# crlotwhite/pytorch_hmm

Hardware: AMD Instinct MI355X
Metric: frames/sec forward-backward+Viterbi, B=32 T=2000 N=128, 1/2/4/8 GPU (higher is better)
Workload: dtype f32; 1 GPU; HMMPyTorch forward_backward + viterbi_decode; batch_per_gpu=32, global_batch=32, seq_len=2000, num_states=128, transition=left_to_right(0.7), world_size_seen=1, parallelism=batch-sharded x1, streams=2, gather=False, hip_graph=False, step_pipelining=per-op streams, no per-step join, transition_plan=True, fb_kernel=chains + posterior followers in one launch, viterbi_kernel=chains + log leaders + decode followers in one launch

## Files before the change

include/hmm355.h:

```cpp
#ifndef HMM355_H
#define HMM355_H

#include <stddef.h>
#include <stdint.h>

#ifdef __cplusplus
extern "C" {
#endif

#define HMM355_OK 0
#define HMM355_E_ARG (-1)
#define HMM355_E_STATES (-2)
#define HMM355_E_SHAPE (-3)
#define HMM355_E_WORKSPACE (-4)
#define HMM355_E_DURATION (-5)

#define HMM355_OBS_PROB 0
#define HMM355_OBS_LOG 1

#define HMM355_FB_POSTERIOR 1u
#define HMM355_FB_FORWARD 2u
#define HMM355_FB_BACKWARD 4u
#define HMM355_FB_PAIR 0x100u
#define HMM355_FB_PLAN_BANDED 0x200u

const char* hmm355_strerror(int code);
int hmm355_version(void);

size_t hmm355_fb_workspace_bytes(int B, int T, int N);
int hmm355_fb_workspace_layout(int B, int T, int N, size_t* offsets);
int hmm355_forward_backward_ex_f32(const float* obs, int obs_mode, const float* log_P,
                                   const float* log_p0, const float* log_beta_T, int B, int T, int N,
                                   unsigned out_mask, float* posterior, float* forward,
                                   float* backward, float* loglik, float* lik_ref, void* workspace,
                                   size_t workspace_bytes, void* stream);
int hmm355_forward_backward_f32(const float* obs, int obs_mode, const float* log_P,
                                const float* log_p0, int B, int T, int N, unsigned out_mask,
                                float* posterior, float* forward, float* backward,
                                float* loglik, float* lik_ref, void* workspace,
                                size_t workspace_bytes, void* stream);

int hmm355_fb_adjoint_f32(const float* E, const float* log_P, const float* src_w,
                          const float* scale_w, const float* src_z, const float* scale_z,
                          int B, int T, int N, float* W, float* P, void* stream);

size_t hmm355_plan_bytes(int N);
int hmm355_plan_f32(const float* log_P, int N, void* plan, void* stream);
// ... 143 lines not shown
```

pytorch_hmm_amd/_native.py:

```python
import ctypes
import os

import torch

_HERE = os.path.dirname(os.path.abspath(__file__))
LIB_PATH = os.environ.get("HMM355_LIB", os.path.join(_HERE, "lib", "libhmm355.so"))

OBS_PROB = 0
OBS_LOG = 1
FB_POSTERIOR = 1
FB_PAIR = 0x100
FB_PLAN_BANDED = 0x200
VIT_PLAN_BANDED = 0x1
VIT_PLAN_DENSE = 0x2
PLAN_DENSE = 0x1
FORM_GENERAL = 0x1
FORM_SERIAL_WALK = 0x2
FB_FORWARD = 2
FB_BACKWARD = 4
NARROW_MAX_STATES = 256
WIDE_MAX_STATES = 4096
DTW_SYMMETRIC, DTW_ASYMMETRIC, DTW_RABINER_JUANG = 0, 1, 2
DTW_PATH = 0x1
CTC_ALPHA, CTC_BETA, CTC_VITERBI = 0x1, 0x2, 0x4
CTC_MAX_TARGET = 2048

EXPORTS = (
    "hmm355_strerror", "hmm355_version",
    "hmm355_fb_workspace_bytes", "hmm355_fb_workspace_layout", "hmm355_forward_backward_f32",
    "hmm355_forward_backward_ex_f32",
    "hmm355_viterbi_workspace_bytes", "hmm355_viterbi_workspace_bytes_ex", "hmm355_viterbi_f32",
    "hmm355_gmm_workspace_bytes", "hmm355_gmm_diag_logprob_f32",
    "hmm355_hsmm_workspace_bytes", "hmm355_hsmm_viterbi_f32", "hmm355_hsmm_workspace_bytes_ex",
    "hmm355_hsmm_viterbi_ex_f32",
    "hmm355_tv_fb_workspace_bytes", "hmm355_tv_forward_backward_f32", "hmm355_tv_forward_backward_ex_f32",
# ... 130 lines not shown
```

pytorch_hmm_amd/csrc/capi.hip:

```cpp
#include "common.h"

HMM355_API int hmm355_version(void) { return 4; }

HMM355_API const char* hmm355_strerror(int code) {
  switch (code) {
    case HMM355_OK: return "ok";
    case HMM355_E_ARG: return "invalid argument (null pointer, negative size or unknown mode)";
    case HMM355_E_STATES: return "number of states outside the op's range (HMM recursions [1, 256], their *_wide forms [1, 4096], HSMM [1, 1024], CTC target length [1, 2048])";
    case HMM355_E_SHAPE: return "invalid shape (T < 1, a DTW matrix without rows or columns, or size overflow)";
    case HMM355_E_WORKSPACE: return "workspace too small";
    case HMM355_E_DURATION: return "HSMM max_duration outside [1, 1024]";
    default: break;
  }
  if (code > 0) return hipGetErrorString(static_cast<hipError_t>(code));
  return "unknown hmm355 error";
}
```

pytorch_hmm_amd/csrc/fb.hip:

```cpp
#include <atomic>

#include "recur.h"
#include "post.h"
#include "fbpair.h"

namespace hmm355 {

template <int NP>
hipError_t launch_fb(const RecArgs& fa, const RecArgs& fb, const PostArgs& pa, bool prep, hipStream_t st, int nfollow);
template <int NP>
hipError_t launch_fb_pair(const PairArgs& pa, int B, hipStream_t st);
__global__ void __launch_bounds__(256) row_max_kernel(const float* __restrict__ lo, int N, size_t rows,
                                                      float* __restrict__ m) {
  const int l = threadIdx.x & 63;
  const size_t nw = ((size_t)gridDim.x * blockDim.x) >> 6;
  for (size_t row = ((size_t)blockIdx.x * blockDim.x + threadIdx.x) >> 6; row < rows; row += nw) {
    const float* src = lo + row * N;
    float v = -INFINITY;
    for (int j = l; j < N; j += 64) v = fmaxf(v, src[j]);
    v = wave_max_dpp2(v);
    if (l == 0) m[row] = (v > -INFINITY && v < INFINITY) ? v : 0.f;
  }
}

// ... 129 lines not shown
    const hipError_t e1 = hipGetLastError();
    if (e1 != hipSuccess) return (int)e1;
    rmax = w.rmax;
  }
  RecArgs fa{obs, log_P, log_p0, w.U, w.LA, loglik, B, T, N, obs_mode, NP, band, nullptr, nullptr, nullptr, rmax, nullptr};
  RecArgs fb{obs, log_P, log_p0, w.V, w.LB, nullptr, B, T, N, obs_mode, NP, band, binit, bscale, nullptr, rmax, nullptr};
  fa.cs = w.CA;
  fb.cs = w.CB;
  hipStream_t st0 = static_cast<hipStream_t>(stream);
  if ((out_mask & HMM355_FB_PAIR) && plan && band && NP <= 128 && !log_beta_T &&
      (size_t)T * NP * sizeof(float) < ((size_t)1 << 31)) {
    PairArgs pa{fa, fb, posterior, forward, backward, lik_ref, out_mask};
    const hipError_t e = NP == 64 ? launch_fb_pair<64>(pa, B, st0) : launch_fb_pair<128>(pa, B, st0);
    return e == hipSuccess ? HMM355_OK : (int)e;
  }
  fa.out_exp = (out_mask & HMM355_FB_FORWARD) ? forward : nullptr;
  fb.out_exp = (out_mask & HMM355_FB_BACKWARD) ? backward : nullptr;
  int nfollow = 0;
  if ((out_mask & HMM355_FB_PLAN_BANDED) && plan && (out_mask & HMM355_FB_POSTERIOR) && 3 * B <= fb_device_cus() &&
      (size_t)T * NP * 4 < ((size_t)1 << 31)) {
    fa.pub = fb.pub = w.pub;
    fa.lik_ref = lik_ref;
    nfollow = HMM355_FBF > 0 ? HMM355_FBF : (4 * B <= fb_device_cus() ? 2 : 1);
  }
  PostArgs pa{w.U, w.V, w.LA, w.LB, posterior, forward, backward, lik_ref, B, T, N,
              out_mask & (HMM355_FB_POSTERIOR)};
  hipError_t e;
  switch (NP) {
    case 64: e = launch_fb<64>(fa, fb, pa, plan == nullptr, st, nfollow); break;
    case 128: e = launch_fb<128>(fa, fb, pa, plan == nullptr, st, nfollow); break;
    default: e = launch_fb<256>(fa, fb, pa, plan == nullptr, st, nfollow); break;
  }
  return e == hipSuccess ? HMM355_OK : (int)e;
}

HMM355_API int hmm355_forward_backward_ex_f32(const float* obs, int obs_mode, const float* log_P,
                                              const float* log_p0, const float* log_beta_T, int B, int T, int N,
                                              unsigned out_mask, float* posterior, float* forward, float* backward,
                                              float* loglik, float* lik_ref, void* workspace,
                                              size_t workspace_bytes, void* stream) {
  return hmm355_forward_backward_plan_f32(obs, obs_mode, log_P, log_p0, nullptr, log_beta_T, B, T, N, out_mask,
                                          posterior, forward, backward, loglik, lik_ref, workspace,
                                          workspace_bytes, stream);
}

HMM355_API int hmm355_forward_backward_f32(const float* obs, int obs_mode, const float* log_P,
// ... 9 lines not shown
```

pytorch_hmm_amd/csrc/follow.h:

```cpp
#pragma once
#include "recur.h"
#include "post.h"

namespace hmm355 {

constexpr long long kFollowGiveUp = 20000000;

__device__ __forceinline__ void fstamp(int k) {
  if (kStamp && threadIdx.x == 0)
    g_rec_stamps[((size_t)blockIdx.x * 16 % kStampWaves) * 8 + k] = __builtin_amdgcn_s_memrealtime();
}

__device__ __forceinline__ void follow_poll(const int* p, int need, int* slot, unsigned token, int cap) {
  int have = poll_count(p, token, cap), last = have;
  long long t0 = __builtin_amdgcn_s_memrealtime();
  while (have < need) {
    __builtin_amdgcn_s_sleep(20);
    have = poll_count(p, token, cap);
    const long long now = __builtin_amdgcn_s_memrealtime();
    if (have != last) {
      last = have;
      t0 = now;
    } else if (now - t0 > kFollowGiveUp) {
      have = -1;
      break;
    }
  }
  *slot = have;
}

template <int NP>
__device__ __forceinline__ void vit_lead(const RecArgs& a, int b) {
  const int T = a.T, N = a.N, nblocks = (T + 15) / 16;
  if (!a.lobuf || nblocks <= 4 || (kFAbl & (fabl::kNoFollowers | fabl::kNoLogLeaders))) return;
  const int tid = threadIdx.x, nt = blockDim.x;
  const size_t off = (size_t)b * T * N;
  const float* src = a.obs + off;
  float* dst = const_cast<float*>(a.lobuf) + off;
  int* cnt = const_cast<int*>(a.lready) + b * kPubStride;
  const __amdgpu_buffer_rsrc_t rs = make_rsrc(dst, (size_t)T * N * 4);
  const bool vec = (N & 3) == 0 && ((reinterpret_cast<uintptr_t>(src) | reinterpret_cast<uintptr_t>(dst)) & 15) == 0;
  constexpr int kRound = 8;
  for (int k0 = 4; k0 < nblocks; k0 += kRound) {
    const int k1 = k0 + kRound < nblocks ? k0 + kRound : nblocks;
    const int e0 = 16 * k0 * N, e1 = (16 * k1 < T ? 16 * k1 : T) * N;
    if (vec) {
      for (int i0 = e0 / 4 + tid; i0 < e1 / 4; i0 += 4 * nt) {
        float4 v[4];
#pragma unroll
        for (int k = 0; k < 4; ++k) {
          const int i = i0 + k * nt;
          v[k] = reinterpret_cast<const float4*>(src)[i < e1 / 4 ? i : i0];
        }
#pragma unroll
        for (int k = 0; k < 4; ++k) {
          const int i = i0 + k * nt;
          const float4 o = make_float4(logcr_fast(v[k].x + 1e-8f, g_logcr_tab), logcr_fast(v[k].y + 1e-8f, g_logcr_tab),
                                       logcr_fast(v[k].z + 1e-8f, g_logcr_tab), logcr_fast(v[k].w + 1e-8f, g_logcr_tab));
          if (i < e1 / 4) __builtin_amdgcn_raw_buffer_store_b128(__builtin_bit_cast(u32x4_t, o), rs, i * 16, 0, kAuxSc1);
        }
      }
    } else {
      for (int i = e0 + tid; i < e1; i += nt)
        __builtin_amdgcn_raw_buffer_store_b32(__builtin_bit_cast(unsigned, logcr_fast(src[i] + 1e-8f, g_logcr_tab)), rs,
                                              i * 4, 0, kAuxSc1);
    }
    asm volatile("s_waitcnt vmcnt(0)" ::: "memory");
    __syncthreads();
    if (tid == 0) publish_count(cnt, k1, a.token);
  }
}

__host__ __device__ constexpr int follow_g(int NP) { return 1024 / NP < 8 ? 1024 / NP : 8; }
inline size_t vit_follow_lds_bytes(int T, int NP) {
  const size_t nc = (T + kChunk - 1) / kChunk;
  return align_up(nc * NP, 16) + (size_t)follow_g(NP) * kChunk * NP + align_up(nc, 4) * 4 + 64;
}

template <int NP>
__device__ __forceinline__ void vit_decode_follow(const RecArgs& a, int b, float* ldsf) {
  const int T = a.T, N = a.N, nblocks = (T + 15) / 16, nc = (T + kChunk - 1) / kChunk;
  const int tid = threadIdx.x, w = __builtin_amdgcn_readfirstlane(tid >> 6), l = tid & 63, nw = blockDim.x >> 6;
  uint8_t* lds = reinterpret_cast<uint8_t*>(ldsf);
  uint8_t* gm = lds;
  uint8_t* stg = gm + align_up((size_t)nc * NP, 16);
  int* send = reinterpret_cast<int*>(stg + (size_t)follow_g(NP) * kChunk * NP);
  int* ctl = send + align_up((size_t)nc, 4);
  int64_t* sb = a.states + (size_t)b * T;
  auto invalid = [&]() {
    for (int t = tid; t < T; t += blockDim.x) sb[t] = -1;
    if (tid == 0 && a.final_score) a.final_score[b] = __builtin_bit_cast(float, 0x7fc00000u);
  };
  fstamp(0);
  if (kFAbl & fabl::kNoFollowers) return;
  if (rec_band_code<kVit, NP>(a) == 0) {
    invalid();
    return;
  }
  const int* pubp = a.pub + b * kPubStride;
  const __amdgpu_buffer_rsrc_t psi_rs = make_rsrc(a.psi + (size_t)b * T * NP, (size_t)T * NP);
  constexpr int G = follow_g(NP);
  int have = 0;
  int next = 0;
  auto wait_for = [&](int need) -> bool {
    if (tid == 0) follow_poll(pubp, need, ctl, a.token, nblocks + 1);
    __syncthreads();
    const int v = ctl[0];
    __syncthreads();
    if (v < 0) return false;
    have = v;
    return true;
  };
  uint8_t* const pbase = a.path + (size_t)b * nc * NP * kChunk;
  auto compose = [&](int c_end) {
    while (next < c_end) {
      const int cnt = c_end - next < G ? c_end - next : G;
      const int per = kChunk * NP / 16;
      for (int idx = tid; idx < cnt * per; idx += blockDim.x) {
        const int g = idx / per, pc = idx - g * per;
        const int t = (next + g) * kChunk + pc / (NP / 16);
        const u32x4_t v = t < T ? __builtin_amdgcn_raw_buffer_load_b128(psi_rs, (t * NP) + 16 * (pc % (NP / 16)), 0, kAuxSc1)
                                : u32x4_t{0u, 0u, 0u, 0u};
        *reinterpret_cast<u32x4_t*>(stg + (size_t)g * kChunk * NP + 16 * pc) = v;
      }
      __syncthreads();
      const int g = tid / NP, j = tid % NP;
      if (g < cnt) {
        const int c = next + g;
        const int t_lo = c * kChunk, t_hi = (t_lo + kChunk < T ? t_lo + kChunk : T) - 1;
        const int len = t_hi - t_lo;
        const uint8_t* pr = stg + (size_t)g * kChunk * NP;
        int st = j < N ? j : 0;
        unsigned acc[kChunk / 4];
        static_for<0, kChunk>([&](auto KK) {
          constexpr int k = kChunk - 1 - decltype(KK)::value;
          if constexpr ((k & 3) == 3) acc[k >> 2] = (unsigned)st << 24;
          else acc[k >> 2] |= (unsigned)st << (8 * (k & 3));
          if constexpr (k >= 1) {
            const int nx = pr[k * NP + st];
            st = k <= len ? nx : st;
          }
        });
        gm[(size_t)c * NP + j] = pr[st];
        uint8_t* dst = pbase + ((size_t)c * NP + j) * kChunk;
#pragma unroll
        for (int q = 0; q < kChunk / 16; ++q)
          *reinterpret_cast<u32x4_t*>(dst + 16 * q) = u32x4_t{acc[4 * q], acc[4 * q + 1], acc[4 * q + 2], acc[4 * q + 3]};
      }
      next += cnt;
      asm volatile("s_waitcnt vmcnt(0)" ::: "memory");
      __syncthreads();
    }
  };
  while (next < nc) {
    const int need = 4 * (next + 1) < nblocks ? 4 * (next + 1) : nblocks;
    if (have < need && !wait_for(need)) {
      invalid();
      return;
    }
    int c_end = have > nblocks ? nc : have / 4;
    if (c_end > nc) c_end = nc;
    if (c_end <= next) c_end = next + 1;
    compose(c_end);
  }
  if (have <= nblocks && !wait_for(nblocks + 1)) {
    invalid();
    return;
  }
  fstamp(1);
  if (w == 0) {
    const float* dl = a.rows + ((size_t)b * T + T - 1) * a.row_stride;
    float bv = -INFINITY;
    int bi = 0x7fffffff;
#pragma unroll
    for (int k = 0; k < NP / 64; ++k) {
      const int j = l + 64 * k;
      const float v = __hip_atomic_load(dl + (j < N ? j : 0), __ATOMIC_RELAXED, __HIP_MEMORY_SCOPE_AGENT);
      if (j < N) argmax_combine(bv, bi, v, j);
    }
    wave_argmax_dpp(bv, bi);
    if (l == 0 && a.final_score) a.final_score[b] = bv;
    int s = bi < N ? bi : 0;
    if (l == 0) send[nc - 1] = s;
    for (int c = nc - 1; c >= 1; --c) {
      s = gm[(size_t)c * NP + s];
      if (l == 0) send[c - 1] = s;
    }
  }
  __syncthreads();
  fstamp(2);
  const __amdgpu_buffer_rsrc_t path_rs = make_rsrc(pbase, (size_t)nc * NP * kChunk);
  for (int idx = tid; idx < nc * (kChunk / 4); idx += blockDim.x) {
    const int c = idx / (kChunk / 4), q = idx % (kChunk / 4);
    const int t0 = c * kChunk + 4 * q;
    if (t0 < T) {
      const unsigned word = __builtin_amdgcn_raw_buffer_load_b32(path_rs, (c * NP + send[c]) * kChunk + 4 * q, 0, kAuxSc1);
#pragma unroll
      for (int i = 0; i < 4; ++i)
        if (t0 + i < T) sb[t0 + i] = (int64_t)((word >> (8 * i)) & 0xffu);
    }
  }
  if (kStamp) {
    __syncthreads();
    fstamp(3);
  }
// ... 11 lines not shown
  float* pbase = posterior + (size_t)b * T * N;
  auto invalid = [&]() {
    for (size_t i = tid; i < (size_t)T * N; i += blockDim.x) pbase[i] = __builtin_bit_cast(float, 0x7fc00000u);
    if (tid == 0 && fa.lik_ref) fa.lik_ref[b] = __builtin_bit_cast(float, 0x7fc00000u);
  };
  fstamp(0);
  if (kFAbl & fabl::kNoFollowers) return;
  if (rec_band_code<kFbAlpha, NP>(fa) == 0 || rec_band_code<kFbBeta, NP>(fb) == 0) {
    invalid();
    return;
  }
  const int* pa = fa.pub + 2 * b * kPubStride;
  const int* pb_ = pa + kPubStride;
  const __amdgpu_buffer_rsrc_t rU = make_rsrc(fa.rows + (size_t)b * T * NP, (size_t)T * NP * 4);
  const __amdgpu_buffer_rsrc_t rV = make_rsrc(fb.rows + (size_t)b * T * NP, (size_t)T * NP * 4);
  const bool vec = N == NP && (reinterpret_cast<uintptr_t>(posterior) % (4 * K)) == 0;
  auto rows_of = [&](int c) { return c > nblocks ? T : (16 * c < T ? 16 * c : T); };
  constexpr int R = HMM355_FBR;
  auto rows = [&](const int (&t)[R], int nv) {
    float u[R][K], v[R][K];
#pragma unroll
    for (int r = 0; r < R; ++r) {
      const int tr = r < nv ? t[r] : t[0];
      if constexpr (K == 1) {
        u[r][0] = __builtin_bit_cast(float, __builtin_amdgcn_raw_buffer_load_b32(rU, (tr * NP + l) * 4, 0, kAuxSc1));
        v[r][0] = __builtin_bit_cast(float, __builtin_amdgcn_raw_buffer_load_b32(rV, (tr * NP + l) * 4, 0, kAuxSc1));
      } else if constexpr (K == 2) {
        const float2 x = __builtin_bit_cast(float2, __builtin_amdgcn_raw_buffer_load_b64(rU, (tr * NP + 2 * l) * 4, 0, kAuxSc1));
        const float2 y = __builtin_bit_cast(float2, __builtin_amdgcn_raw_buffer_load_b64(rV, (tr * NP + 2 * l) * 4, 0, kAuxSc1));
        u[r][0] = x.x; u[r][1] = x.y; v[r][0] = y.x; v[r][1] = y.y;
      } else {
        const float4 x = __builtin_bit_cast(float4, __builtin_amdgcn_raw_buffer_load_b128(rU, (tr * NP + 4 * l) * 4, 0, kAuxSc1));
        const float4 y = __builtin_bit_cast(float4, __builtin_amdgcn_raw_buffer_load_b128(rV, (tr * NP + 4 * l) * 4, 0, kAuxSc1));
        u[r][0] = x.x; u[r][1] = x.y; u[r][2] = x.z; u[r][3] = x.w;
        v[r][0] = y.x; v[r][1] = y.y; v[r][2] = y.z; v[r][3] = y.w;
      }
    }
#pragma unroll
    for (int r = 0; r < R; ++r) {
      if (r >= nv) break;
      const int t_ = t[r];
      float mu = 0.f, mv = 0.f;
#pragma unroll
      for (int k = 0; k < K; ++k) { mu = fmaxf(mu, u[r][k]); mv = fmaxf(mv, v[r][k]); }
      mu = wave_max_dpp2(mu);
      mv = wave_max_dpp2(mv);
      const float iu = mu > 0.f ? 1.f / mu : 0.f, iv = mv > 0.f ? 1.f / mv : 0.f;
      float p[K], sum = 0.f;
#pragma unroll
      for (int k = 0; k < K; ++k) { p[k] = (u[r][k] * iu) * (v[r][k] * iv); sum += p[k]; }
      sum = wave_sum_dpp(sum);
      const float is = sum > 0.f ? 1.f / sum : 0.f;
#pragma unroll
      for (int k = 0; k < K; ++k) p[k] *= is;
      if (vec) {
        float* dst = pbase + (size_t)t_ * N + K * l;
        if constexpr (K == 1) dst[0] = p[0];
        else if constexpr (K == 2) *reinterpret_cast<float2*>(dst) = make_float2(p[0], p[1]);
        else *reinterpret_cast<float4*>(dst) = make_float4(p[0], p[1], p[2], p[3]);
      } else {
#pragma unroll
        for (int k = 0; k < K; ++k)
          if (K * l + k < N) pbase[(size_t)t_ * N + K * l + k] = p[k];
      }
    }
  };
  int plo = -1, phi = -1;
  int ca = 0, cb = 0;
  while (plo != 0 || phi != T) {
    if (tid == 0) {
      int ok = 1;
      long long t0 = __builtin_amdgcn_s_memrealtime();
      for (;;) {
        const int na = poll_count(pa, fa.token, nblocks + 1), nb = poll_count(pb_, fa.token, nblocks + 1);
        const int lo = T - rows_of(nb), hi = rows_of(na);
        const bool more = lo < hi && (plo < 0 || lo < plo || hi > phi);
        if (more) { ca = na; cb = nb; break; }
        if (na != ca || nb != cb) { ca = na; cb = nb; t0 = __builtin_amdgcn_s_memrealtime(); }
        else if (__builtin_amdgcn_s_memrealtime() - t0 > kFollowGiveUp) { ok = 0; break; }
        __builtin_amdgcn_s_sleep(20);
      }
      ctl[0] = ok; ctl[1] = ca; ctl[2] = cb;
    }
    __syncthreads();
    const int ok = ctl[0];
    ca = ctl[1];
    cb = ctl[2];
    __syncthreads();
    if (!ok) {
      invalid();
      return;
    }
    if (kStamp && ca > nblocks && cb > nblocks) fstamp(1);
    const int lo = T - rows_of(cb), hi = rows_of(ca);
    const int a0 = first_own(lo), a1 = plo < 0 ? hi : plo;
    const int b0 = first_own(plo < 0 ? hi : phi), b1 = hi;
    const int na = a1 > a0 ? (a1 - a0 + F - 1) / F : 0;
    const int nn = na + (b1 > b0 ? (b1 - b0 + F - 1) / F : 0);
    for (int i0 = w * R; i0 < nn; i0 += nw * R) {
      int t[R];
#pragma unroll
      for (int r = 0; r < R; ++r) t[r] = i0 + r < na ? a0 + F * (i0 + r) : b0 + F * (i0 + r - na);
      rows(t, nn - i0 < R ? nn - i0 : R);
    }
    plo = lo;
    phi = hi;
  }
  if (kStamp) {
    __syncthreads();
    fstamp(2);
  }
}

}
```

pytorch_hmm_amd/csrc/post.h:

```cpp
#pragma once
#include <type_traits>
#include "common.h"
#include "band.h"

namespace hmm355 {

struct PostArgs {
  const float* U;
  const float* V;
  const float* LA;
  const float* LB;
  float* posterior;
  float* forward;
  float* backward;
  float* lik_ref;
  int B, T, N;
  unsigned mask;
};

constexpr int kPostWaves = 32768;

template <int NP>
__global__ void __launch_bounds__(256) fb_posterior_kernel(PostArgs a) {
  constexpr int K = NP / 64;
  using VecK = typename std::conditional<K == 1, float, typename std::conditional<K == 2, float2, float4>::type>::type;
  const int l = threadIdx.x & 63;
  const int wave = (blockIdx.x * blockDim.x + threadIdx.x) >> 6;
  const int nwaves = (gridDim.x * blockDim.x) >> 6;
  const size_t rows = (size_t)a.B * a.T;
  const bool vec = a.N == NP && (reinterpret_cast<uintptr_t>(a.posterior) | reinterpret_cast<uintptr_t>(a.forward) |
                                 reinterpret_cast<uintptr_t>(a.backward)) % sizeof(VecK) == 0;
  auto jof = [&](int k) { return vec ? K * l + k : l + 64 * k; };
  auto load = [&](size_t row, float (&u)[K], float (&v)[K], float& la, float& lb) {
    if (vec) {
      const VecK tu = reinterpret_cast<const VecK*>(a.U + row * NP)[l];
      const VecK tv = reinterpret_cast<const VecK*>(a.V + row * NP)[l];
      __builtin_memcpy(u, &tu, sizeof(tu));
      __builtin_memcpy(v, &tv, sizeof(tv));
    } else {
#pragma unroll
      for (int k = 0; k < K; ++k) {
// ... 209 lines not shown
```

pytorch_hmm_amd/csrc/recur.h:

```cpp
#pragma once
#include "band.h"
#include "common.h"
#include "logcr.h"

namespace hmm355 {

enum RecKind : int { kFbAlpha = 0, kFbBeta = 1, kVit = 2 };

constexpr int kStampWaves = 512 * 16;
static __device__ unsigned long long g_rec_stamps[kStamp ? kStampWaves * 8 : 1];

template <int NP>
struct RC {
  static constexpr int NW = NP / 16;
  static constexpr int NT = NW * kWave;
  static constexpr int NBLK = NP / 64;
  static constexpr int RING = 64;
  static constexpr int OFF_PART = 0;
  static constexpr int OFF_EMIS = OFF_PART + 2 * NP * 2;
  static constexpr int OFF_RING = OFF_EMIS + 3 * 16 * NP;
  static constexpr int OFF_SC = OFF_RING + RING * NP;
  static constexpr int OFF_M = OFF_SC + RING * 64;
  static constexpr int MRING = 128;
  static constexpr int OFF_LOGT = OFF_M + MRING;
  static constexpr int LDS_FLOATS = OFF_LOGT + 512;
  static_assert(LDS_FLOATS * 4 <= kExclusiveLds, "LDS layout too large");
  static constexpr int PSR = 64;
  static constexpr int OFF_PSR = LDS_FLOATS;
  static_assert((OFF_PSR + PSR * NP / 4) * 4 <= kExclusiveLds, "fused Viterbi LDS layout too large");
};

template <int NP>
struct kRbHelpers {
  static constexpr int NH = NP <= 128 ? RC<NP>::NW / 2 : 0;
  static constexpr int NT = RC<NP>::NT + NH * kWave;
  static_assert(NH <= 8, "kProgSlots");
};
template <int NP>
constexpr int kFbNT = kRbHelpers<NP>::NT;

template <bool MAX, int L>
__device__ __forceinline__ float wave_red_level(float x) {
  constexpr int CTRL = L == 0 ? 0xB1 : L == 1 ? 0x4E : L == 2 ? 0x124 : L == 3 ? 0x128 : L == 4 ? 0x142 : 0x143;
  const float o = __builtin_bit_cast(
      float, __builtin_amdgcn_update_dpp(0, __builtin_bit_cast(int, x), CTRL, 0xF, 0xF, L >= 4));
  return MAX ? fmaxf(x, o) : x + o;
}
__device__ __forceinline__ float wave_lane63(float x) {
  return __builtin_bit_cast(float, __builtin_amdgcn_readlane(__builtin_bit_cast(int, x), 63));
// ... 214 lines not shown
  float* rows;
  float* ls;
  float* loglik;
  int B, T, N, obs_mode, row_stride;
  const BandDesc* band;
  const float* binit;
  const float* bscale;
  uint8_t* psi;
  const float* rmax;
  float* out_exp;
  uint8_t* G;
  int64_t* states;
  float* final_score;
  int nchunks;
  int* prog;
  uint8_t* done;
  float* cs;
  int* pub;
  const float* lobuf;
  const int* lready;
  float* lik_ref;
  uint8_t* path;
  unsigned token;
};
constexpr int kProgSlots = 8;

constexpr int kPsiChunk = 64;
template <int NP>
constexpr bool kVitFused = RC<NP>::NW >= 6;
template <int NP>
constexpr int kVitNT = kVitFused<NP> ? (1024 > kRbHelpers<NP>::NT ? 1024 : kRbHelpers<NP>::NT)
                                     : kRbHelpers<NP>::NT;

template <int KIND>
__device__ __forceinline__ int rec_tau(int q, int T) {
  return KIND == kFbBeta ? T - 1 - q : q;
}

__device__ const double g_logcr_tab[256] = {HMM355_LOGCR_TABLE};
template <int NP>
__device__ __forceinline__ void rec_logt_fill(float* lds, int l) {
  double* t = reinterpret_cast<double*>(lds + RC<NP>::OFF_LOGT);
#pragma unroll
  for (int k = 0; k < 4; ++k) t[l + 64 * k] = g_logcr_tab[l + 64 * k];
}

// ... 973 lines not shown
            if constexpr (NB == 2) *reinterpret_cast<uint16_t*>(ldst) = (uint16_t)pk;
            else *reinterpret_cast<uint32_t*>(ldst) = pk;
          }
        }
      }
    };
    const bool pubon = a.pub != nullptr;
    int* const pubp = pubon ? a.pub + (FB ? 2 * b + (KIND == kFbBeta) : b) * kPubStride : nullptr;
    [[maybe_unused]] const __amdgpu_buffer_rsrc_t psi_rs =
        FUSE ? make_rsrc(a.psi + (size_t)b * T * NP, (size_t)T * NP) : make_rsrc(a.obs, 0);
    [[maybe_unused]] auto psi_copy = [&](int bk) {
      if constexpr (FUSE) {
        constexpr int PER = NP / 16;
        const int hidx = (NH - 1 - hi) * 64 + l;
        const int r = hidx / PER, pc = hidx % PER;
        const int t = 16 * bk + r;
        const u32x4_t v = *reinterpret_cast<const u32x4_t*>(reinterpret_cast<const uint8_t*>(lds + C::OFF_PSR) +
                                                            (t & (C::PSR - 1)) * NP + 16 * pc);
        if (bk >= 0 && hidx < 16 * PER && t < T)
          __builtin_amdgcn_raw_buffer_store_b128(v, psi_rs, t * NP + 16 * pc, 0, (kFAbl & fabl::kPlainStores) ? 0 : kAuxSc1);
      }
    };
    unsigned long long hs_work = 0, hs_wait = 0;
    auto block_work = [&](int kb, float(&ernext)[HV][5], float(&erfree)[HV][5], int& lp, auto FULLC) {
      asm volatile("" ::: "memory");
      unsigned long long hs0 = 0;
      if (kStamp) hs0 = stamp();
      const int kload = kb + 3 < nblocks ? kb + 3 : nblocks - 1;
      float lsv = 0.f;
      if (!(kAbl & abl::kBandNoFlush) && kb >= 2) lsv = rec_ls_scan<NP, KIND>(a, lds, b, kb - 2, base, w == 1);
      const bool fromlog = KIND == kVit && a.lobuf && kload >= 4 && lp >= kload + 1;
      const float* src = fromlog ? a.lobuf : a.obs;
      const float vmode = (fromlog || a.obs_mode == HMM355_OBS_LOG) ? 1.f : 0.f;
#pragma unroll
      for (int h = 0; h < HV; ++h) {
        const int vw = vw_of(h);
        if (vw < C::NW && !(kAbl & abl::kBandNoHelperWork)) {
          if (!(kAbl & abl::kBandNoStage)) {
            rec_stage<NP, KIND, FUSE>(a, lds, kb + 1, vw, l, ernext[h]);
            rec_load<NP, KIND, decltype(FULLC)::value, FUSE>(a, b, kload, vw, l, erfree[h], src, vmode);
          }
          if (!(kAbl & abl::kBandNoFlush) && kb >= 2) rec_flush<NP, KIND>(a, lds, b, kb - 2, l + 64 * vw, lsv);
        }
      }
      psi_copy(kb - 3);
      if (KIND == kVit && a.lready) lp = poll_count(a.lready + b * kPubStride, a.token, nblocks);
      if (pubon && !(kFAbl & fabl::kNoBlockPublish) && hi == 0 && l == 0) {
        const int cnt = FB ? kb - 5 : kb - 6;
        if (cnt > 0 && (cnt & 3) == 0) publish_count(pubp, cnt, a.token);
      }
      unsigned long long hs1 = 0;
      if (kStamp) { hs1 = stamp(); hs_work += hs1 - hs0; }
      if (!(kAbl & abl::kBandNoBlockBarrier)) lds_barrier();
      if (kStamp) hs_wait += stamp() - hs1;
    };
    if constexpr (FUSE) {
      if (psiw) {
        for (int kb = 0; kb < nblocks; ++kb) {
          psi_rows(kb - 2);
          if (!(kAbl & abl::kBandNoBlockBarrier)) lds_barrier();
        }
        lds_barrier();
        psi_rows(nblocks - 2);
        psi_rows(nblocks - 1);
        lds_barrier();
        return;
      }
    }
    int lp0 = 0, lp1 = 0, lp2 = 0;
    auto helper_loop = [&](auto FULLC) {
      for (int kb = 0; kb < nblocks; kb += 3) {
        block_work(kb, er1, er0, lp0, FULLC);
        if (kb + 1 < nblocks) block_work(kb + 1, er2, er1, lp1, FULLC);
        if (kb + 2 < nblocks) block_work(kb + 2, er0, er2, lp2, FULLC);
      }
    };
    if (a.N == NP && (reinterpret_cast<uintptr_t>(a.obs) & 15) == 0 &&
        (!a.lobuf || (reinterpret_cast<uintptr_t>(a.lobuf) & 15) == 0))
      helper_loop(std::true_type{});
    else
      helper_loop(std::false_type{});
    if (kStamp && l == 0 && stager) {
      unsigned long long* o8 = g_rec_stamps + (((size_t)blockIdx.x * 16 + w) % kStampWaves) * 8;
      o8[0] = hs_work; o8[1] = hs_wait; o8[4] = (unsigned long long)nblocks;
    }
    lds_barrier();
    if (FB && pubon && nblocks > 6) {
      asm volatile("s_waitcnt vmcnt(0)" ::: "memory");
      __syncthreads();
      if (hi == 0 && l == 0) publish_count(pubp, nblocks - 2, a.token);
    }
    const float lsv2 = nblocks >= 2 ? rec_ls_scan<NP, KIND>(a, lds, b, nblocks - 2, base, w == 1) : 0.f;
    const float lsv1 = rec_ls_scan<NP, KIND>(a, lds, b, nblocks - 1, base, w == 1);
    if (FB && pubon) {
#pragma unroll
      for (int h = 0; h < HV; ++h) {
        const int vw = vw_of(h);
        if (vw < C::NW) {
          if (nblocks >= 2) rec_flush<NP, KIND, 1>(a, lds, b, nblocks - 2, l + 64 * vw, lsv2);
          rec_flush<NP, KIND, 1>(a, lds, b, nblocks - 1, l + 64 * vw, lsv1);
        }
      }
      asm volatile("s_waitcnt vmcnt(0)" ::: "memory");
      __syncthreads();
      if (hi == 0 && l == 0) publish_count(pubp, nblocks + 1, a.token);
      if (kStamp && hi == 0 && l == 0) g_rec_stamps[((size_t)blockIdx.x * 16 % kStampWaves) * 8 + 2] = __builtin_amdgcn_s_memrealtime();
    }
#pragma unroll
    for (int h = 0; h < HV; ++h) {
      const int vw = vw_of(h);
      if (vw < C::NW) {
        if (FB && pubon) {
          if (nblocks >= 2) rec_flush<NP, KIND, 2>(a, lds, b, nblocks - 2, l + 64 * vw, lsv2);
          rec_flush<NP, KIND, 2>(a, lds, b, nblocks - 1, l + 64 * vw, lsv1);
        } else {
          if (nblocks >= 2) rec_flush<NP, KIND>(a, lds, b, nblocks - 2, l + 64 * vw, lsv2);
          rec_flush<NP, KIND>(a, lds, b, nblocks - 1, l + 64 * vw, lsv1);
        }
        if (KIND == kFbAlpha && a.loglik && vw == C::NW - 1 && l == 0)
          a.loglik[b] = rec_loglik<NP>(lds, T, base);
      }
    }
    if constexpr (KIND == kFbAlpha) {
      if (a.lik_ref && hi == 0) {
        const float ls = __shfl(lsv1, (T - 1) & 15);
// ... 4 lines not shown
          const int j = l + 64 * k;
          lv[k] = j < N ? __logf(__expf(__logf(u[j]) + ls) + 1e-8f) : -INFINITY;
          m = fmaxf(m, lv[k]);
        }
        m = wave_max(m);
        float e = 0.f;
#pragma unroll
        for (int k = 0; k < NB; ++k) e += (l + 64 * k < N) ? __expf(lv[k] - m) : 0.f;
        e = wave_sum(e);
        if (l == 0) a.lik_ref[b] = m + __logf(e);
      }
    }
    if constexpr (FUSE) {
      psi_copy(nblocks - 3);
      lds_barrier();
      psi_copy(nblocks - 2);
      psi_copy(nblocks - 1);
    }
    if (!FB && pubon) {
      asm volatile("s_waitcnt vmcnt(0)" ::: "memory");
      __syncthreads();
      if (hi == 0 && l == 0) publish_count(pubp, nblocks + 1, a.token);
      if (kStamp && hi == 0 && l == 0) g_rec_stamps[((size_t)blockIdx.x * 16 % kStampWaves) * 8 + 2] = __builtin_amdgcn_s_memrealtime();
    }
}

template <int KIND, int NP>
__device__ __forceinline__ int rec_band_code(const RecArgs& a) {
  if (!a.band) return 0;
  const BandDesc* d = a.band;
  const int W = KIND == kFbBeta ? d->wr : d->wc;
  if (W > kBandMax) return 0;
  const int tw = KIND == kFbBeta ? d->trw : d->tcw;
  const int td0 = KIND == kFbBeta ? d->trd0 : d->tcd0;
  if (NP <= 128 && tw > 0) {
    const int code = 16 * tw + td0 + 2;
    switch (code) {
      case 16 * 1 + 0 + 2: case 16 * 2 - 1 + 2: case 16 * 2 + 0 + 2:
      case 16 * 3 - 2 + 2: case 16 * 3 - 1 + 2: case 16 * 3 + 0 + 2: return code;
      default: break;
    }
  }
  return KIND == kFbBeta ? d->wrp : d->wcp;
}

template <int NP, int KIND>
// ... 28 lines not shown
```

pytorch_hmm_amd/csrc/vit_kern.h:

```cpp
#pragma once
#include "recur.h"
#include "post.h"
#include "follow.h"

namespace hmm355 {


template <int NP>
__device__ __forceinline__ void vit_psi_follow(const RecArgs& ra, float* lds);

template <int NP>
__global__ void __launch_bounds__(kVitNT<NP>) vit_fwd_kernel(RecArgs ra) {
  extern __shared__ __attribute__((aligned(16))) float lds[];
  if ((int)blockIdx.x >= ra.B) {
    if (ra.pub) {
      if constexpr (kVitFused<NP>) {
        const int b = (int)blockIdx.x - ra.B;
        vit_lead<NP>(ra, b);
        vit_decode_follow<NP>(ra, b, lds);
      }
      return;
    }
    if constexpr (NP <= 128) vit_psi_follow<NP>(ra, lds);
    return;
// ... 257 lines not shown
  }
}

template <int NP>
hipError_t launch_vit(const VitArgs& va, bool prep, hipStream_t sm) {
  hipError_t e = allow_lds(vit_fwd_kernel<NP>, kExclusiveLds);
  if (e != hipSuccess) return e;
  if (va.band && prep) {
    e = launch_band_prep(va.log_P, va.N, const_cast<BandDesc*>(va.band), sm);
    if (e != hipSuccess) return e;
  }
  RecArgs ra{va.obs, va.log_P, va.init, va.delta, nullptr, nullptr, va.B, va.T, va.N, va.obs_mode, va.N, va.band,
             nullptr, nullptr, va.psi};
  ra.G = va.G;
  ra.states = va.states;
  ra.final_score = va.final_score;
  ra.nchunks = va.nchunks;
  if (va.pub) {
    ra.pub = va.pub;
    ra.lobuf = va.lobuf;
    ra.lready = va.lready;
    ra.path = va.path;
    ra.token = va.token;
    hipLaunchKernelGGL(vit_fwd_kernel<NP>, dim3(2 * va.B), dim3(kVitNT<NP>), kExclusiveLds, sm, ra);
    return hipGetLastError();
  }
  const int nfollow = (NP <= 128 && va.prog && va.done) ? va.nfollow : 0;
  if (nfollow > 0) {
    e = zero_words(va.prog, (size_t)va.B * kProgSlots * sizeof(int), sm);
    if (e == hipSuccess) e = zero_words(va.done, (size_t)va.B * va.nchunks, sm);
    if (e != hipSuccess) return e;
    ra.prog = va.prog;
    ra.done = va.done;
  }
  hipLaunchKernelGGL(vit_fwd_kernel<NP>, dim3(va.B + nfollow), dim3(kVitNT<NP>), kExclusiveLds, sm, ra);
  e = hipGetLastError();
  if (e != hipSuccess) return e;
  const size_t psi_lds = va.band ? (size_t)kChunk * NP * sizeof(float) : 0;
  VitArgs vp = va;
  if (nfollow == 0) vp.done = nullptr;
  hipLaunchKernelGGL(vit_psi_kernel<NP>, dim3(va.nchunks, va.B), dim3(VF<NP>::NT), psi_lds, sm, vp);
  e = hipGetLastError();
  if (e != hipSuccess) return e;
  hipLaunchKernelGGL(vit_backtrace_kernel<NP>, dim3(va.nchunks, va.B), dim3(64), 0, sm, va);
  return hipGetLastError();
}
// ... 3 lines not shown
```

pytorch_hmm_amd/ops.py:

```python
from typing import Optional, Tuple

import torch
from torch import Tensor

from . import _native as nat

OBS_PROB = nat.OBS_PROB
OBS_LOG = nat.OBS_LOG
FB_POSTERIOR = nat.FB_POSTERIOR
FB_PAIR = nat.FB_PAIR
FB_PLAN_BANDED = nat.FB_PLAN_BANDED
VIT_PLAN_BANDED = nat.VIT_PLAN_BANDED
VIT_PLAN_DENSE = nat.VIT_PLAN_DENSE
FORM_GENERAL = nat.FORM_GENERAL
FORM_SERIAL_WALK = nat.FORM_SERIAL_WALK
FB_FORWARD = nat.FB_FORWARD
FB_BACKWARD = nat.FB_BACKWARD
NARROW_MAX_STATES = nat.NARROW_MAX_STATES
WIDE_MAX_STATES = nat.WIDE_MAX_STATES

_EMPTY = (0,)


def _f32c(t):
    return t.to(torch.float32).contiguous()


def _workspace(nbytes, device):
    return torch.empty(max(int(nbytes), 1), dtype=torch.uint8, device=device)


def _use_wide(N: int, wide: Optional[bool]) -> bool:
    return N > NARROW_MAX_STATES if wide is None else bool(wide)

# ... 685 lines not shown
```

Measured before the change: 378.5 million frames/s.

## Compute end-row posteriors in chain blocks and stream Viterbi backtrack table

The forward and backward chain blocks now compute posterior rows for the last two blocks of each direction themselves, using the opposite chain's published rows, so the follower blocks stop earlier and only pick up rows flagged as left over. Counts are published every block near the end of the chain. The fused Viterbi chain also publishes the final argmax and score through a tagged 64-bit word. The decode follower builds an incremental backpointer composition table in LDS as chunks arrive, so the final backtrack becomes a table lookup instead of a serial walk. The aim is to shorten the tail latency after the recurrences finish, at the cost of more polling, LDS use and more complex synchronisation.

```diff
diff --git a/include/hmm355.h b/include/hmm355.h
--- a/include/hmm355.h
+++ b/include/hmm355.h
@@ -23,6 +23,8 @@
 #define HMM355_FB_BACKWARD 4u
 #define HMM355_FB_PAIR 0x100u
 #define HMM355_FB_PLAN_BANDED 0x200u
+#define HMM355_FB_NO_END_ROWS 0x400u
+#define HMM355_FB_END_ROWS_ODD_LEFT 0x800u
 
 const char* hmm355_strerror(int code);
 int hmm355_version(void);
diff --git a/pytorch_hmm_amd/_native.py b/pytorch_hmm_amd/_native.py
--- a/pytorch_hmm_amd/_native.py
+++ b/pytorch_hmm_amd/_native.py
@@ -11,6 +11,8 @@
 FB_POSTERIOR = 1
 FB_PAIR = 0x100
 FB_PLAN_BANDED = 0x200
+FB_NO_END_ROWS = 0x400
+FB_END_ROWS_ODD_LEFT = 0x800
 VIT_PLAN_BANDED = 0x1
 VIT_PLAN_DENSE = 0x2
 PLAN_DENSE = 0x1
diff --git a/pytorch_hmm_amd/csrc/capi.hip b/pytorch_hmm_amd/csrc/capi.hip
--- a/pytorch_hmm_amd/csrc/capi.hip
+++ b/pytorch_hmm_amd/csrc/capi.hip
@@ -1,6 +1,6 @@
 #include "common.h"
 
-HMM355_API int hmm355_version(void) { return 4; }
+HMM355_API int hmm355_version(void) { return 5; }
 
 HMM355_API const char* hmm355_strerror(int code) {
   switch (code) {
diff --git a/pytorch_hmm_amd/csrc/fb.hip b/pytorch_hmm_amd/csrc/fb.hip
--- a/pytorch_hmm_amd/csrc/fb.hip
+++ b/pytorch_hmm_amd/csrc/fb.hip
@@ -175,6 +175,12 @@
     fa.pub = fb.pub = w.pub;
     fa.lik_ref = lik_ref;
     nfollow = HMM355_FBF > 0 ? HMM355_FBF : (4 * B <= fb_device_cus() ? 2 : 1);
+    if (T >= kEndMinT && !(out_mask & HMM355_FB_NO_END_ROWS)) {
+      fa.ends = fb.ends = kEndsOn | ((out_mask & HMM355_FB_END_ROWS_ODD_LEFT) ? kEndsOddLeft : 0u);
+      fa.prow = w.V;
+      fb.prow = w.U;
+      fa.post = fb.post = posterior;
+    }
   }
   PostArgs pa{w.U, w.V, w.LA, w.LB, posterior, forward, backward, lik_ref, B, T, N,
               out_mask & (HMM355_FB_POSTERIOR)};
diff --git a/pytorch_hmm_amd/csrc/follow.h b/pytorch_hmm_amd/csrc/follow.h
--- a/pytorch_hmm_amd/csrc/follow.h
+++ b/pytorch_hmm_amd/csrc/follow.h
@@ -27,6 +27,36 @@
     }
   }
   *slot = have;
+}
+
+__device__ __forceinline__ void follow_poll_end(const int* p, int need, int* slot, unsigned token, int nblocks) {
+  const unsigned tag = vit_end_tag(token);
+  unsigned long long e = 0;
+  auto poll = [&]() -> int {
+    const unsigned long long* pe = reinterpret_cast<const unsigned long long*>(p + kVitEndWord);
+    const unsigned long long ev = __hip_atomic_load(pe, __ATOMIC_RELAXED, __HIP_MEMORY_SCOPE_AGENT);
+    const int c = poll_count(p, token, nblocks + 1);
+    if (c <= nblocks) return c;
+    e = ev;
+    return ((unsigned)ev >> 8) == tag ? c : nblocks;
+  };
+  int have = poll(), last = have;
+  long long t0 = __builtin_amdgcn_s_memrealtime();
+  while (have < need) {
+    __builtin_amdgcn_s_sleep(20);
+    have = poll();
+    const long long now = __builtin_amdgcn_s_memrealtime();
+    if (have != last) {
+      last = have;
+      t0 = now;
+    } else if (now - t0 > kFollowGiveUp) {
+      have = -1;
+      break;
+    }
+  }
+  slot[0] = have;
+  slot[1] = (int)((unsigned)e & 0xffu);
+  slot[2] = (int)(unsigned)(e >> 32);
 }
 
 template <int NP>
@@ -72,9 +102,10 @@
 }
 
 __host__ __device__ constexpr int follow_g(int NP) { return 1024 / NP < 8 ? 1024 / NP : 8; }
-inline size_t vit_follow_lds_bytes(int T, int NP) {
+inline size_t vit_follow_lds_bytes(int T, int NP, bool table = false) {
   const size_t nc = (T + kChunk - 1) / kChunk;
-  return align_up(nc * NP, 16) + (size_t)follow_g(NP) * kChunk * NP + align_up(nc, 4) * 4 + 64;
+  return align_up(nc * NP, 16) + (size_t)follow_g(NP) * kChunk * NP + align_up(nc, 4) * 4 + 64 +
+         (table ? 2 * (size_t)NP * align_up(nc, 4) : 0);
 }
 
 template <int NP>
@@ -86,6 +117,10 @@
   uint8_t* stg = gm + align_up((size_t)nc * NP, 16);
   int* send = reinterpret_cast<int*>(stg + (size_t)follow_g(NP) * kChunk * NP);
   int* ctl = send + align_up((size_t)nc, 4);
+  const bool tab = a.vit_table != 0;
+  const int ncp = (int)align_up((size_t)nc, 4), nq = ncp / 4;
+  unsigned* const stab = reinterpret_cast<unsigned*>(ctl + 16);
+  int scur = 0;
   int64_t* sb = a.states + (size_t)b * T;
   auto invalid = [&]() {
     for (int t = tid; t < T; t += blockDim.x) sb[t] = -1;
@@ -102,10 +137,16 @@
   constexpr int G = follow_g(NP);
   int have = 0;
   int next = 0;
+  int end_state = 0;
+  float end_score = 0.f;
   auto wait_for = [&](int need) -> bool {
-    if (tid == 0) follow_poll(pubp, need, ctl, a.token, nblocks + 1);
+    if (tid == 0) follow_poll_end(pubp, need, ctl, a.token, nblocks);
     __syncthreads();
     const int v = ctl[0];
+    if (v > nblocks) {
+      end_state = ctl[1];
+      end_score = __builtin_bit_cast(float, ctl[2]);
+    }
     __syncthreads();
     if (v < 0) return false;
     have = v;
@@ -150,6 +191,22 @@
       next += cnt;
       asm volatile("s_waitcnt vmcnt(0)" ::: "memory");
       __syncthreads();
+      if (tab) {
+        for (int c = next - cnt < 1 ? 1 : next - cnt; c < next; ++c) {
+          const unsigned* src = stab + (size_t)scur * NP * nq;
+          unsigned* dst = stab + (size_t)(scur ^ 1) * NP * nq;
+          const int nd = (c - 1) / 4 + 1, sh = 8 * ((c - 1) & 3);
+          for (int idx = tid; idx < NP * nd; idx += blockDim.x) {
+            const int j = idx / nd, d = idx - j * nd;
+            const unsigned g = gm[(size_t)c * NP + j];
+            unsigned wv = src[g * nq + d];
+            if (d == nd - 1) wv = (wv & ~(0xffu << sh)) | (g << sh);
+            dst[j * nq + d] = wv;
+          }
+          scur ^= 1;
+          __syncthreads();
+        }
+      }
     }
   };
   while (next < nc) {
@@ -168,19 +225,13 @@
     return;
   }
   fstamp(1);
-  if (w == 0) {
-    const float* dl = a.rows + ((size_t)b * T + T - 1) * a.row_stride;
-    float bv = -INFINITY;
-    int bi = 0x7fffffff;
-#pragma unroll
-    for (int k = 0; k < NP / 64; ++k) {
-      const int j = l + 64 * k;
-      const float v = __hip_atomic_load(dl + (j < N ? j : 0), __ATOMIC_RELAXED, __HIP_MEMORY_SCOPE_AGENT);
-      if (j < N) argmax_combine(bv, bi, v, j);
-    }
-    wave_argmax_dpp(bv, bi);
-    if (l == 0 && a.final_score) a.final_score[b] = bv;
-    int s = bi < N ? bi : 0;
+  const int send_last = (unsigned)end_state < (unsigned)N ? end_state : 0;
+  if (tid == 0 && a.final_score) a.final_score[b] = end_score;
+  if (tab) {
+    const uint8_t* srow = reinterpret_cast<const uint8_t*>(stab + ((size_t)scur * NP + send_last) * nq);
+    for (int c = tid; c < nc; c += blockDim.x) send[c] = c == nc - 1 ? send_last : srow[c];
+  } else if (w == 0) {
+    int s = send_last;
     if (l == 0) send[nc - 1] = s;
     for (int c = nc - 1; c >= 1; --c) {
       s = gm[(size_t)c * NP + s];
@@ -238,58 +289,27 @@
 #pragma unroll
     for (int r = 0; r < R; ++r) {
       const int tr = r < nv ? t[r] : t[0];
-      if constexpr (K == 1) {
-        u[r][0] = __builtin_bit_cast(float, __builtin_amdgcn_raw_buffer_load_b32(rU, (tr * NP + l) * 4, 0, kAuxSc1));
-        v[r][0] = __builtin_bit_cast(float, __builtin_amdgcn_raw_buffer_load_b32(rV, (tr * NP + l) * 4, 0, kAuxSc1));
-      } else if constexpr (K == 2) {
-        const float2 x = __builtin_bit_cast(float2, __builtin_amdgcn_raw_buffer_load_b64(rU, (tr * NP + 2 * l) * 4, 0, kAuxSc1));
-        const float2 y = __builtin_bit_cast(float2, __builtin_amdgcn_raw_buffer_load_b64(rV, (tr * NP + 2 * l) * 4, 0, kAuxSc1));
-        u[r][0] = x.x; u[r][1] = x.y; v[r][0] = y.x; v[r][1] = y.y;
-      } else {
-        const float4 x = __builtin_bit_cast(float4, __builtin_amdgcn_raw_buffer_load_b128(rU, (tr * NP + 4 * l) * 4, 0, kAuxSc1));
-        const float4 y = __builtin_bit_cast(float4, __builtin_amdgcn_raw_buffer_load_b128(rV, (tr * NP + 4 * l) * 4, 0, kAuxSc1));
-        u[r][0] = x.x; u[r][1] = x.y; u[r][2] = x.z; u[r][3] = x.w;
-        v[r][0] = y.x; v[r][1] = y.y; v[r][2] = y.z; v[r][3] = y.w;
-      }
+      post_row_load<K>(rU, tr, l, u[r]);
+      post_row_load<K>(rV, tr, l, v[r]);
     }
 #pragma unroll
     for (int r = 0; r < R; ++r) {
       if (r >= nv) break;
-      const int t_ = t[r];
-      float mu = 0.f, mv = 0.f;
-#pragma unroll
-      for (int k = 0; k < K; ++k) { mu = fmaxf(mu, u[r][k]); mv = fmaxf(mv, v[r][k]); }
-      mu = wave_max_dpp2(mu);
-      mv = wave_max_dpp2(mv);
-      const float iu = mu > 0.f ? 1.f / mu : 0.f, iv = mv > 0.f ? 1.f / mv : 0.f;
-      float p[K], sum = 0.f;
-#pragma unroll
-      for (int k = 0; k < K; ++k) { p[k] = (u[r][k] * iu) * (v[r][k] * iv); sum += p[k]; }
-      sum = wave_sum_dpp(sum);
-      const float is = sum > 0.f ? 1.f / sum : 0.f;
-#pragma unroll
-      for (int k = 0; k < K; ++k) p[k] *= is;
-      if (vec) {
-        float* dst = pbase + (size_t)t_ * N + K * l;
-        if constexpr (K == 1) dst[0] = p[0];
-        else if constexpr (K == 2) *reinterpret_cast<float2*>(dst) = make_float2(p[0], p[1]);
-        else *reinterpret_cast<float4*>(dst) = make_float4(p[0], p[1], p[2], p[3]);
-      } else {
-#pragma unroll
-        for (int k = 0; k < K; ++k)
-          if (K * l + k < N) pbase[(size_t)t_ * N + K * l + k] = p[k];
-      }
-    }
-  };
+      post_row_lanes<K>(u[r], v[r], pbase + (size_t)t[r] * N, N, l, vec);
+    }
+  };
+  const bool ends = (fa.ends & kEndsOn) != 0;
+  const int qend0 = 16 * (nblocks - kEndBlocks), nend = T - qend0;
+  const int rlo = ends ? nend : 0, rhi = ends ? qend0 : T;
   int plo = -1, phi = -1;
   int ca = 0, cb = 0;
-  while (plo != 0 || phi != T) {
+  while (plo != rlo || phi != rhi) {
     if (tid == 0) {
       int ok = 1;
       long long t0 = __builtin_amdgcn_s_memrealtime();
       for (;;) {
         const int na = poll_count(pa, fa.token, nblocks + 1), nb = poll_count(pb_, fa.token, nblocks + 1);
-        const int lo = T - rows_of(nb), hi = rows_of(na);
+        const int lo = max(T - rows_of(nb), rlo), hi = min(rows_of(na), rhi);
         const bool more = lo < hi && (plo < 0 || lo < plo || hi > phi);
         if (more) { ca = na; cb = nb; break; }
         if (na != ca || nb != cb) { ca = na; cb = nb; t0 = __builtin_amdgcn_s_memrealtime(); }
@@ -308,7 +328,7 @@
       return;
     }
     if (kStamp && ca > nblocks && cb > nblocks) fstamp(1);
-    const int lo = T - rows_of(cb), hi = rows_of(ca);
+    const int lo = max(T - rows_of(cb), rlo), hi = min(rows_of(ca), rhi);
     const int a0 = first_own(lo), a1 = plo < 0 ? hi : plo;
     const int b0 = first_own(plo < 0 ? hi : phi), b1 = hi;
     const int na = a1 > a0 ? (a1 - a0 + F - 1) / F : 0;
@@ -322,6 +342,40 @@
     plo = lo;
     phi = hi;
   }
+  if (ends) {
+    if (tid == 0) {
+      follow_poll(pa + kLeftWord, (int)kLeftValid, ctl + 1, fa.token, (int)kLeftCap);
+      follow_poll(pb_ + kLeftWord, (int)kLeftValid, ctl + 2, fa.token, (int)kLeftCap);
+      int ok = ctl[1] >= 0 && ctl[2] >= 0;
+      if (ok && ((ctl[1] | ctl[2]) & (int)(kLeftValid - 1u))) {
+        follow_poll(pa, nblocks + 1, ctl, fa.token, nblocks + 1);
+        ok = ctl[0] >= 0;
+        if (ok) {
+          follow_poll(pb_, nblocks + 1, ctl, fa.token, nblocks + 1);
+          ok = ctl[0] >= 0;
+        }
+      }
+      ctl[0] = ok;
+    }
+    __syncthreads();
+    const int ok = ctl[0], left[2] = {ctl[1], ctl[2]};
+    __syncthreads();
+    if (!ok) {
+      invalid();
+      return;
+    }
+    if (kStamp) fstamp(1);
+    if ((left[0] | left[1]) & (int)(kLeftValid - 1u)) {
+      for (int i = w; i < 2 * nend; i += nw) {
+        const int d = i / nend, q = qend0 + i % nend;
+        const int tq = d ? T - 1 - q : q;
+        if (((left[d] >> (nblocks - 1 - (q >> 4))) & 1) && tq % F == f) {
+          const int t[R] = {tq};
+          rows(t, 1);
+        }
+      }
+    }
+  }
   if (kStamp) {
     __syncthreads();
     fstamp(2);
diff --git a/pytorch_hmm_amd/csrc/post.h b/pytorch_hmm_amd/csrc/post.h
--- a/pytorch_hmm_amd/csrc/post.h
+++ b/pytorch_hmm_amd/csrc/post.h
@@ -17,6 +17,57 @@
   int B, T, N;
   unsigned mask;
 };
+
+template <int K>
+__device__ __forceinline__ void post_row_lanes(const float (&u)[K], const float (&v)[K], float* dst, int N, int l, bool vec,
+                                               bool on = true) {
+  float mu = 0.f, mv = 0.f;
+#pragma unroll
+  for (int k = 0; k < K; ++k) { mu = fmaxf(mu, u[k]); mv = fmaxf(mv, v[k]); }
+  mu = wave_max_dpp2(mu);
+  mv = wave_max_dpp2(mv);
+  const float iu = mu > 0.f ? 1.f / mu : 0.f, iv = mv > 0.f ? 1.f / mv : 0.f;
+  float p[K], sum = 0.f;
+#pragma unroll
+  for (int k = 0; k < K; ++k) { p[k] = (u[k] * iu) * (v[k] * iv); sum += p[k]; }
+  sum = wave_sum_dpp(sum);
+  const float is = sum > 0.f ? 1.f / sum : 0.f;
+#pragma unroll
+  for (int k = 0; k < K; ++k) p[k] *= is;
+  if (!on) return;
+  if (vec) {
+    if constexpr (K == 1) dst[l] = p[0];
+    else if constexpr (K == 2) *reinterpret_cast<float2*>(dst + 2 * l) = make_float2(p[0], p[1]);
+    else *reinterpret_cast<float4*>(dst + 4 * l) = make_float4(p[0], p[1], p[2], p[3]);
+  } else {
+#pragma unroll
+    for (int k = 0; k < K; ++k)
+      if (K * l + k < N) dst[K * l + k] = p[k];
+  }
+}
+template <int K>
+__device__ __forceinline__ void post_row_load(const __amdgpu_buffer_rsrc_t rs, int t, int l, float (&x)[K]) {
+  const int off = (t * 64 * K + K * l) * 4;
+  if constexpr (K == 1) {
+    x[0] = __builtin_bit_cast(float, __builtin_amdgcn_raw_buffer_load_b32(rs, off, 0, kAuxSc1));
+  } else if constexpr (K == 2) {
+    const float2 y = __builtin_bit_cast(float2, __builtin_amdgcn_raw_buffer_load_b64(rs, off, 0, kAuxSc1));
+    x[0] = y.x; x[1] = y.y;
+  } else {
+    const float4 y = __builtin_bit_cast(float4, __builtin_amdgcn_raw_buffer_load_b128(rs, off, 0, kAuxSc1));
+    x[0] = y.x; x[1] = y.y; x[2] = y.z; x[3] = y.w;
+  }
+}
+
+constexpr int kEndBlocks = 2;
+constexpr int kEndMinT = 256;
+constexpr int kLateBlocks = 12;
+constexpr unsigned kEndsOn = 1u, kEndsOddLeft = 2u;
+constexpr int kLeftWord = 2;
+constexpr unsigned kLeftValid = 0x8000u, kLeftCap = 0xffffu;
+
+constexpr int kVitEndWord = 2;
+__device__ __forceinline__ unsigned vit_end_tag(unsigned token) { return ((count_mix(token) >> 8) | 1u) & 0xffffffu; }
 
 constexpr int kPostWaves = 32768;
 
diff --git a/pytorch_hmm_amd/csrc/recur.h b/pytorch_hmm_amd/csrc/recur.h
--- a/pytorch_hmm_amd/csrc/recur.h
+++ b/pytorch_hmm_amd/csrc/recur.h
@@ -2,6 +2,7 @@
 #include "band.h"
 #include "common.h"
 #include "logcr.h"
+#include "post.h"
 
 namespace hmm355 {
 
@@ -25,6 +26,8 @@
   static constexpr int OFF_LOGT = OFF_M + MRING;
   static constexpr int LDS_FLOATS = OFF_LOGT + 512;
   static_assert(LDS_FLOATS * 4 <= kExclusiveLds, "LDS layout too large");
+  static constexpr int OFF_LEFT = LDS_FLOATS;
+  static_assert((OFF_LEFT + 16) * 4 <= kExclusiveLds, "end-row LDS layout too large");
   static constexpr int PSR = 64;
   static constexpr int OFF_PSR = LDS_FLOATS;
   static_assert((OFF_PSR + PSR * NP / 4) * 4 <= kExclusiveLds, "fused Viterbi LDS layout too large");
@@ -285,6 +288,10 @@
   float* lik_ref;
   uint8_t* path;
   unsigned token;
+  const float* prow;
+  float* post;
+  unsigned ends;
+  int vit_table;
 };
 constexpr int kProgSlots = 8;
 
@@ -1304,6 +1311,61 @@
       }
     };
     unsigned long long hs_work = 0, hs_wait = 0;
+    constexpr int KL = NP / 64;
+    constexpr int RE = (16 * kEndBlocks + NH - 1) / NH;
+    [[maybe_unused]] float epr[RE][KL];
+    [[maybe_unused]] int eok = 0;
+    const bool endson = FB && stager && pubon && (a.ends & kEndsOn) && a.prow && a.post;
+    const int qend0 = 16 * (nblocks - kEndBlocks);
+    auto end_row = [&](int m, int& q) -> bool {
+      q = qend0 + hi + NH * m;
+      return q < T;
+    };
+    [[maybe_unused]] auto end_load = [&]() {
+      if constexpr (FB) {
+        const int* ppub = a.pub + (2 * b + (KIND == kFbAlpha)) * kPubStride;
+        const int cnt = __builtin_amdgcn_readfirstlane(poll_count(ppub, a.token, nblocks + 1));
+        const bool counted = cnt > nblocks || 16 * cnt >= T - qend0;
+        int leftmask = 0;
+#pragma unroll
+        for (int m = 0; m < RE; ++m) {
+          int q;
+          const bool live = end_row(m, q);
+          const bool ok = counted && !((a.ends & kEndsOddLeft) && ((q >> 4) & 1));
+          eok |= (int)ok << m;
+          if (live && !ok) leftmask |= 1 << (nblocks - 1 - (q >> 4));
+          int tq = live ? rec_tau<KIND>(q, T) : 0;
+          asm volatile("" : "+v"(tq) : "s"(cnt));
+          post_row_load<KL>(make_rsrc(a.prow + (size_t)b * T * NP, (size_t)T * NP * 4), tq, l, epr[m]);
+        }
+        if (l == 0) reinterpret_cast<int*>(lds + C::OFF_LEFT)[hi] = leftmask;
+      }
+    };
+    [[maybe_unused]] auto end_post = [&]() {
+      if constexpr (FB) {
+        const bool endvec = N == NP && (reinterpret_cast<uintptr_t>(a.post) % (4 * KL)) == 0;
+#pragma unroll
+        for (int m = 0; m < RE; ++m) {
+          int q;
+          const bool on = end_row(m, q) && ((eok >> m) & 1);
+          const int tq = on ? rec_tau<KIND>(q, T) : 0;
+          float own[KL];
+          const float* rp = lds + C::OFF_RING + (q & (C::RING - 1)) * NP + KL * l;
+          if constexpr (KL == 1) {
+            own[0] = rp[0];
+          } else if constexpr (KL == 2) {
+            const float2 y = *reinterpret_cast<const float2*>(rp);
+            own[0] = y.x; own[1] = y.y;
+          } else {
+            const float4 y = *reinterpret_cast<const float4*>(rp);
+            own[0] = y.x; own[1] = y.y; own[2] = y.z; own[3] = y.w;
+          }
+          float* dst = a.post + ((size_t)b * T + tq) * N;
+          if (KIND == kFbAlpha) post_row_lanes<KL>(own, epr[m], dst, N, l, endvec, on);
+          else post_row_lanes<KL>(epr[m], own, dst, N, l, endvec, on);
+        }
+      }
+    };
     auto block_work = [&](int kb, float(&ernext)[HV][5], float(&erfree)[HV][5], int& lp, auto FULLC) {
       asm volatile("" ::: "memory");
       unsigned long long hs0 = 0;
@@ -1329,7 +1391,8 @@
       if (KIND == kVit && a.lready) lp = poll_count(a.lready + b * kPubStride, a.token, nblocks);
       if (pubon && !(kFAbl & fabl::kNoBlockPublish) && hi == 0 && l == 0) {
         const int cnt = FB ? kb - 5 : kb - 6;
-        if (cnt > 0 && (cnt & 3) == 0) publish_count(pubp, cnt, a.token);
+        const bool late = FB && (a.ends & kEndsOn) && kb >= nblocks - kLateBlocks;
+        if (cnt > 0 && ((cnt & 3) == 0 || late)) publish_count(pubp, cnt, a.token);
       }
       unsigned long long hs1 = 0;
       if (kStamp) { hs1 = stamp(); hs_work += hs1 - hs0; }
@@ -1366,7 +1429,32 @@
       unsigned long long* o8 = g_rec_stamps + (((size_t)blockIdx.x * 16 + w) % kStampWaves) * 8;
       o8[0] = hs_work; o8[1] = hs_wait; o8[4] = (unsigned long long)nblocks;
     }
+    if (endson) end_load();
     lds_barrier();
+    if (endson && hi == 0 && l == 0) {
+      int m = 0;
+      for (int h = 0; h < NH; ++h) m |= reinterpret_cast<const int*>(lds + C::OFF_LEFT)[h];
+      publish_count(const_cast<int*>(pubp) + kLeftWord, m | (int)kLeftValid, a.token);
+    }
+    if constexpr (FUSE) {
+      if (pubon && hi == 0) {
+        const float* dl = lds + C::OFF_RING + ((T - 1) & (C::RING - 1)) * NP;
+        float bv = -INFINITY;
+        int bi = 0x7fffffff;
+#pragma unroll
+        for (int k = 0; k < NP / 64; ++k) {
+          const int j = l + 64 * k;
+          const float v = dl[j];
+          if (j < N) argmax_combine(bv, bi, v, j);
+        }
+        wave_argmax_dpp(bv, bi);
+        if (l == 0)
+          __hip_atomic_store(reinterpret_cast<unsigned long long*>(pubp + kVitEndWord),
+                             ((unsigned long long)__builtin_bit_cast(unsigned, bv) << 32) | (vit_end_tag(a.token) << 8) |
+                                 (unsigned)(bi < N ? bi : 0),
+                             __ATOMIC_RELAXED, __HIP_MEMORY_SCOPE_AGENT);
+      }
+    }
     if (FB && pubon && nblocks > 6) {
       asm volatile("s_waitcnt vmcnt(0)" ::: "memory");
       __syncthreads();
@@ -1383,6 +1471,7 @@
           rec_flush<NP, KIND, 1>(a, lds, b, nblocks - 1, l + 64 * vw, lsv1);
         }
       }
+      if (endson) end_post();
       asm volatile("s_waitcnt vmcnt(0)" ::: "memory");
       __syncthreads();
       if (hi == 0 && l == 0) publish_count(pubp, nblocks + 1, a.token);
@@ -1433,6 +1522,10 @@
       __syncthreads();
       if (hi == 0 && l == 0) publish_count(pubp, nblocks + 1, a.token);
       if (kStamp && hi == 0 && l == 0) g_rec_stamps[((size_t)blockIdx.x * 16 % kStampWaves) * 8 + 2] = __builtin_amdgcn_s_memrealtime();
+    }
+    if (kStamp && hi == 0) {
+      asm volatile("s_waitcnt vmcnt(0)" ::: "memory");
+      if (l == 0) g_rec_stamps[(((size_t)blockIdx.x * 16 + w) % kStampWaves) * 8 + 2] = __builtin_amdgcn_s_memrealtime();
     }
 }
 
diff --git a/pytorch_hmm_amd/csrc/vit_kern.h b/pytorch_hmm_amd/csrc/vit_kern.h
--- a/pytorch_hmm_amd/csrc/vit_kern.h
+++ b/pytorch_hmm_amd/csrc/vit_kern.h
@@ -303,6 +303,7 @@
     ra.lready = va.lready;
     ra.path = va.path;
     ra.token = va.token;
+    ra.vit_table = vit_follow_lds_bytes(va.T, NP, true) <= kExclusiveLds;
     hipLaunchKernelGGL(vit_fwd_kernel<NP>, dim3(2 * va.B), dim3(kVitNT<NP>), kExclusiveLds, sm, ra);
     return hipGetLastError();
   }
diff --git a/pytorch_hmm_amd/ops.py b/pytorch_hmm_amd/ops.py
--- a/pytorch_hmm_amd/ops.py
+++ b/pytorch_hmm_amd/ops.py
@@ -10,6 +10,8 @@
 FB_POSTERIOR = nat.FB_POSTERIOR
 FB_PAIR = nat.FB_PAIR
 FB_PLAN_BANDED = nat.FB_PLAN_BANDED
+FB_NO_END_ROWS = nat.FB_NO_END_ROWS
+FB_END_ROWS_ODD_LEFT = nat.FB_END_ROWS_ODD_LEFT
 VIT_PLAN_BANDED = nat.VIT_PLAN_BANDED
 VIT_PLAN_DENSE = nat.VIT_PLAN_DENSE
 FORM_GENERAL = nat.FORM_GENERAL
```

Measured after the change: 382.7 million frames/s (median of 6 runs). +1.1%, better.
